# cvsp-lab/ICLR2025_3D-MOM

Hardware: AMD Instinct MI355X
Metric: 4DGS train-steps/sec @200k Gaussians, 960×540, 60 frames; render FPS (higher is better)
Workload: dtype f32

## Files before the change

### iclr2025_3d-mom_amd/csrc/hexplane.hip

```cpp
#include "hexplane_dev.h"

namespace {

template <int C> constexpr int kGroups = 64 / C;
template <int C> constexpr unsigned kRowB = 4u * C;
template <int C> constexpr int kPad = C == 16 ? 1 : 0;
constexpr int kChunk = 32;
template <int C> constexpr int kPerGroup = kChunk / kGroups<C>;
template <int C> constexpr int kRecs = kChunk * 6 + kPad<C> * kGroups<C>;
template <int C> __device__ __forceinline__ constexpr int rec_idx(int pt, int p) { return pt * 6 + p + kPad<C> * (pt / kPerGroup<C>); }

template <int C> __device__ __forceinline__ float group_sum(float v)
{
#pragma unroll
    for (int d = C / 2; d >= 1; d >>= 1) v += __shfl_xor(v, d);
    return v;
}

template <int C> __device__ __forceinline__ void norm_coords_fwd(const HexArgs& a, const float* __restrict__ xyz, int g, float c[4])
{
    if constexpr (C == 32) norm_coords_fwd32(a, xyz, g, c);
    else norm_coords(a, xyz, g, c);
}

template <int C>
__global__ void __launch_bounds__(256) hexplane_fwd_kernel(HexArgs a, const float* __restrict__ xyz, float* __restrict__ feat)
{
    const int ch = threadIdx.x & (C - 1);
    const long long unit = (long long)blockIdx.x * (256 / C) + threadIdx.x / C;
    const int gi = (int)(unit / a.levels), lvl = (int)(unit % a.levels);
    if (gi >= a.P) return;
    const int g = a.order ? (int)a.order[gi] : gi;
    float c[4];
    norm_coords_fwd<C>(a, xyz, g, c);
    float prod = 1.f;
#pragma unroll
    for (int p = 0; p < 6; p++) {
        const int ca = kCombA[p], cb = kCombB[p];
        const int Wd = a.res[lvl][ca], Hd = a.res[lvl][cb];
        const PlaneSample s = make_sample(c[ca], c[cb], Wd, Hd);
        const float* __restrict__ pl = a.planes[lvl][p];
        float v = 0.f;
        if (s.i00 >= 0) v += pl[(size_t)s.i00 * C + ch] * s.w00;
        if (s.i01 >= 0) v += pl[(size_t)s.i01 * C + ch] * s.w01;
        if (s.i10 >= 0) v += pl[(size_t)s.i10 * C + ch] * s.w10;
        if (s.i11 >= 0) v += pl[(size_t)s.i11 * C + ch] * s.w11;
        prod = prod * v;
    }
    feat[(size_t)g * (a.levels * C) + lvl * C + ch] = prod;
}

template <int C>
__global__ void __launch_bounds__(256)
hexplane_bwd_kernel(HexArgs a, const float* __restrict__ xyz, const float* __restrict__ dfeat, float* __restrict__ dxyz)
{
    const int ch = threadIdx.x & (C - 1);
    const long long unit = (long long)blockIdx.x * (256 / C) + threadIdx.x / C;
    const int g = (int)(unit / a.levels), lvl = (int)(unit % a.levels);
    if (g >= a.P) return;
    float c[4];
    norm_coords(a, xyz, g, c);
    PlaneSample s[6];
    float v[6], t00[6], t01[6], t10[6], t11[6];
#pragma unroll
    for (int p = 0; p < 6; p++) {
        const int ca = kCombA[p], cb = kCombB[p];
        s[p] = make_sample(c[ca], c[cb], a.res[lvl][ca], a.res[lvl][cb]);
        const float* __restrict__ pl = a.planes[lvl][p];
        t00[p] = s[p].i00 >= 0 ? pl[(size_t)s[p].i00 * C + ch] : 0.f;
        t01[p] = s[p].i01 >= 0 ? pl[(size_t)s[p].i01 * C + ch] : 0.f;
        t10[p] = s[p].i10 >= 0 ? pl[(size_t)s[p].i10 * C + ch] : 0.f;
        t11[p] = s[p].i11 >= 0 ? pl[(size_t)s[p].i11 * C + ch] : 0.f;
        float acc = 0.f;
        acc += t00[p] * s[p].w00;
        acc += t01[p] * s[p].w01;
        acc += t10[p] * s[p].w10;
        acc += t11[p] * s[p].w11;
        v[p] = acc;
    }
    const float go = dfeat[(size_t)g * (a.levels * C) + lvl * C + ch];
    float pre[7], suf[7];
    pre[0] = 1.f;
#pragma unroll
    for (int p = 0; p < 6; p++) pre[p + 1] = pre[p] * v[p];
    suf[6] = 1.f;
#pragma unroll
    for (int p = 5; p >= 0; p--) suf[p] = suf[p + 1] * v[p];
    float gc[3] = {0.f, 0.f, 0.f};
#pragma unroll
    for (int p = 0; p < 6; p++) {
        const float gv = go * pre[p] * suf[p + 1];
        float* __restrict__ gp = a.grads[lvl][p];
        if (s[p].i00 >= 0) atomicAdd(&gp[(size_t)s[p].i00 * C + ch], gv * s[p].w00);
        if (s[p].i01 >= 0) atomicAdd(&gp[(size_t)s[p].i01 * C + ch], gv * s[p].w01);
        if (s[p].i10 >= 0) atomicAdd(&gp[(size_t)s[p].i10 * C + ch], gv * s[p].w10);
        if (s[p].i11 >= 0) atomicAdd(&gp[(size_t)s[p].i11 * C + ch], gv * s[p].w11);
        const float x0 = (float)s[p].ixn, y0 = (float)s[p].iyn, x1 = x0 + 1.f, y1 = y0 + 1.f;
        float gix = 0.f, giy = 0.f;
        gix -= t00[p] * (y1 - s[p].iy) * gv;
        giy -= t00[p] * (x1 - s[p].ix) * gv;
        gix += t01[p] * (y1 - s[p].iy) * gv;
        giy -= t01[p] * (s[p].ix - x0) * gv;
        gix -= t10[p] * (s[p].iy - y0) * gv;
        giy += t10[p] * (x1 - s[p].ix) * gv;
        gix += t11[p] * (s[p].iy - y0) * gv;
        giy += t11[p] * (s[p].ix - x0) * gv;
        const int ca = kCombA[p], cb = kCombB[p];
        if (ca < 3) gc[ca] += gix * s[p].gx_mul;
        if (cb < 3) gc[cb] += giy * s[p].gy_mul;
    }
    if (dxyz) {
#pragma unroll
        for (int k = 0; k < 3; k++) {
            const float tot = group_sum<C>(gc[k]) * (2.0f / (a.a1[k] - a.a0[k]));
            if (ch == 0) atomicAdd(&dxyz[3 * g + k], tot);
        }
    }
}



template <int C>
__device__ __forceinline__ void make_rec_fwd(float cx, float cy, int Wd, int Hd, uint4& O, float4& Wt)
{
    float gxm, gym;
    const float ix = unnorm_clip(cx, Wd, gxm), iy = unnorm_clip(cy, Hd, gym);
    const int x0 = (int)floorf(ix), y0 = (int)floorf(iy);
    const unsigned o00 = (unsigned)(y0 * Wd + x0) * kRowB<C>, sx = (x0 + 1 < Wd) ? kRowB<C> : 0u, sy = (y0 + 1 < Hd) ? (unsigned)Wd * kRowB<C> : 0u;
    const float bx = ix - (float)x0, by = iy - (float)y0, ax = 1.f - bx, ay = 1.f - by;
    O = make_uint4(o00, o00 + sx, o00 + sy, o00 + sy + sx);
    Wt = make_float4(ax * ay, bx * ay, ax * by, bx * by);
}

template <int C>
__global__ void __launch_bounds__(256)
hexplane_fwd4_kernel(HexArgs a, int nchunks, const float* __restrict__ xyz, float* __restrict__ feat)
{
    __shared__ uint4 s_off[4][kRecs<C>];
    __shared__ float4 s_wt[4][kRecs<C>];
    const int lane = threadIdx.x & 63, ch = lane & (C - 1), q = lane / C, wv = threadIdx.x >> 6;
    const int lvl = blockIdx.y;
    const int wave = (blockIdx.x * 256 + threadIdx.x) >> 6, nwaves = (gridDim.x * 256) >> 6;
    for (int chunk = wave; chunk < nchunks; chunk += nwaves) {
        const int gi = chunk * kChunk + lane;
        const int g_mine = (lane < kChunk && gi < a.P) ? (a.order ? (int)a.order[gi] : gi) : -1;
        __builtin_amdgcn_wave_barrier();
        if (g_mine >= 0) {
            float c[4];
            norm_coords_fwd<C>(a, xyz, g_mine, c);
#pragma unroll
            for (int p = 0; p < 6; p++)
                make_rec_fwd<C>(c[kCombA[p]], c[kCombB[p]], a.res[lvl][kCombA[p]], a.res[lvl][kCombB[p]], s_off[wv][rec_idx<C>(lane, p)],
                                s_wt[wv][rec_idx<C>(lane, p)]);
        }
        __builtin_amdgcn_wave_barrier();
        const int npts = min(kChunk, a.P - chunk * kChunk);
        const int n_grp = max(0, min(kPerGroup<C>, npts - kPerGroup<C> * q));
        for (int i = 0; i < n_grp; i++) {
            const int pt = kPerGroup<C> * q + i;
            const int g = __shfl(g_mine, pt);
            float prod = 1.f;
#pragma unroll
            for (int p = 0; p < 6; p++) {
                const uint4 o = s_off[wv][rec_idx<C>(pt, p)];
                const float4 w = s_wt[wv][rec_idx<C>(pt, p)];
                const float* __restrict__ pl = a.planes[lvl][p] + ch;
                float v = 0.f;
                v += ld_f32(pl, o.x) * w.x;
                v += ld_f32(pl, o.y) * w.y;
                v += ld_f32(pl, o.z) * w.z;
                v += ld_f32(pl, o.w) * w.w;
                prod = prod * v;
            }
            feat[(size_t)g * (a.levels * C) + lvl * C + ch] = prod;
        }
    }
}


template <int C>
__device__ __forceinline__ void make_rec5(float cx, float cy, int Wd, int Hd, unsigned row_off, float gsx, float gsy, uint4& R1, float4& R2)
{
    float gxm, gym;
    const float ix = unnorm_clip(cx, Wd, gxm), iy = unnorm_clip(cy, Hd, gym);
    const int x0 = (int)floorf(ix), y0 = (int)floorf(iy);
    R1 = make_uint4((unsigned)(y0 * Wd + x0) * kRowB<C>, (x0 + 1 < Wd) ? kRowB<C> : 0u, (y0 + 1 < Hd) ? (unsigned)Wd * kRowB<C> : 0u, row_off);
    R2 = make_float4(ix - (float)x0, iy - (float)y0, gxm != 0.f ? gsx : 0.f, gym != 0.f ? gsy : 0.f);
}

template <int C>
__global__ void __launch_bounds__(256, 4)
hexplane_bwd5_gather_kernel(HexArgs a, int nchunks, const float* __restrict__ xyz, const float* __restrict__ dfeat,
                            float* __restrict__ dxyz, const uint32_t* __restrict__ inv ,
                            float* __restrict__ gvbuf )
{
    __shared__ uint4 s_r1[4][kRecs<C>];
    __shared__ float4 s_r2[4][kRecs<C>];
    const int lane = threadIdx.x & 63, ch = lane & (C - 1), q = lane / C, wv = threadIdx.x >> 6;
    const int pj = lane & 31, hh = lane >> 5;
    const int lvl = blockIdx.y;
    const int wave = (blockIdx.x * 256 + threadIdx.x) >> 6, nwaves = (gridDim.x * 256) >> 6;
    const unsigned chb = (unsigned)ch * 4u;
    const size_t plane_floats = (size_t)a.P * C;
    float gscale[4];
#pragma unroll
    for (int k = 0; k < 3; k++) gscale[k] = ((float)(a.res[lvl][k] - 1) / 2.f) * (2.0f / (a.a1[k] - a.a0[k]));
    gscale[3] = 0.f;

    for (int chunk = wave; chunk < nchunks; chunk += nwaves) {
        const int gi = chunk * kChunk + pj;
        const int g_mine = gi < a.P ? (a.order ? (int)a.order[gi] : gi) : -1;
        __builtin_amdgcn_wave_barrier();
        if (g_mine >= 0) {
            float c[4];
            norm_coords(a, xyz, g_mine, c);
            unsigned pos[3];
#pragma unroll
            for (int k = 0; k < 3; k++) pos[k] = inv[((size_t)k * a.levels + lvl) * a.P + g_mine] * (2u * kRowB<C>);
#pragma unroll
            for (int r = 0; r < 3; r++) {
                const int p0 = r, p1 = 3 + r;
                const int ca = hh ? kCombA[p1] : kCombA[p0], cb = hh ? kCombB[p1] : kCombB[p0];
                const int slot = hh ? order_slot_of_plane(p1) : order_slot_of_plane(p0);
                uint4 R1; float4 R2;
                make_rec5<C>(c[ca], c[cb], a.res[lvl][ca], a.res[lvl][cb], pos[slot], gscale[ca], gscale[cb], R1, R2);
                s_r1[wv][rec_idx<C>(pj, 3 * hh + r)] = R1;
                s_r2[wv][rec_idx<C>(pj, 3 * hh + r)] = R2;
            }
        }
        __builtin_amdgcn_wave_barrier();
        const int npts = min(kChunk, a.P - chunk * kChunk);
        const int n_grp = max(0, min(kPerGroup<C>, npts - kPerGroup<C> * q));
        const int pt0 = kPerGroup<C> * q;
        float t00[6], t01[6], t10[6], t11[6];
        float go = 0.f;
        float dx_mine[3] = {0.f, 0.f, 0.f};
        auto fetch = [&](int i) {
            const int ng = __shfl(g_mine, pt0 + i);
#pragma unroll
            for (int p = 0; p < 6; p++) {
                const uint4 R1 = s_r1[wv][rec_idx<C>(pt0 + i, p)];
                const float* __restrict__ pl = a.planes[lvl][p];
                const unsigned o = R1.x + chb;
                t00[p] = ld_f32(pl, o);
                t01[p] = ld_f32(pl, o + R1.y);
                t10[p] = ld_f32(pl, o + R1.z);
                t11[p] = ld_f32(pl, o + R1.y + R1.z);
            }
            go = dfeat[(size_t)ng * (a.levels * C) + lvl * C + ch];
        };
        if (n_grp > 0) fetch(0);
        for (int i = 0; i < n_grp; i++) {
            float v[6], dgx[6], dgy[6];
#pragma unroll
            for (int p = 0; p < 6; p++) {
                const float4 R2 = s_r2[wv][rec_idx<C>(pt0 + i, p)];
                const float d0 = t01[p] - t00[p], d1 = t11[p] - t10[p];
                const float tx0 = __builtin_fmaf(R2.x, d0, t00[p]), tx1 = __builtin_fmaf(R2.x, d1, t10[p]);
                const float dy = tx1 - tx0;
                v[p] = __builtin_fmaf(R2.y, dy, tx0);
                dgx[p] = __builtin_fmaf(R2.y, d1 - d0, d0) * R2.z;
                dgy[p] = dy * R2.w;
            }
            const float gcur = go;
            const int icur = i;
            if (i + 1 < n_grp) fetch(i + 1);
            float pre[7], suf[7];
            pre[0] = 1.f;
#pragma unroll
            for (int p = 0; p < 6; p++) pre[p + 1] = pre[p] * v[p];
            suf[6] = 1.f;
#pragma unroll
            for (int p = 5; p >= 0; p--) suf[p] = suf[p + 1] * v[p];
            float gc[3] = {0.f, 0.f, 0.f};
#pragma unroll
            for (int p = 0; p < 6; p++) {
                const float gv = gcur * (pre[p] * suf[p + 1]);
                const int ca = kCombA[p], cb = kCombB[p];
                float* __restrict__ dst = gvbuf + ((size_t)order_slot_of_plane(p) * a.levels + lvl) * 2 * plane_floats + ((p == 2 || p == 4 || p == 5) ? C : 0);
                *reinterpret_cast<float*>(reinterpret_cast<char*>(dst) + (s_r1[wv][rec_idx<C>(pt0 + icur, p)].w + chb)) = gv;
                gc[ca] = __builtin_fmaf(gv, dgx[p], gc[ca]);
                if (cb < 3) gc[cb] = __builtin_fmaf(gv, dgy[p], gc[cb]);
            }
            if (dxyz) {
#pragma unroll
                for (int k = 0; k < 3; k++) {
                    const float tot = group_sum<C>(gc[k]);
                    if (ch == icur) dx_mine[k] = tot;
                }
            }
        }
        if (dxyz) {
            const int gp = __shfl(g_mine, pt0 + (ch & (kPerGroup<C> - 1)));
            if (ch < n_grp && gp >= 0) {
#pragma unroll
                for (int k = 0; k < 3; k++) atomicAdd(&dxyz[3 * gp + k], dx_mine[k]);
            }
        }
    }
}

constexpr int kBatch5s = 16;
constexpr int kRec5s = 4 + 4 + 4 + 2;
template <int C> constexpr int kSlots5s = 64 + kPad<C> * kGroups<C>;

template <int C, bool CROWS>
__global__ void __launch_bounds__(256)
hexplane_bwd5_scatter_kernel(HexArgs a, int per_group, const float* __restrict__ xyz,
                             const uint32_t* __restrict__ order , const float* __restrict__ gvbuf,
                             const float* __restrict__ lines, LineTab lt)
{
    static_assert(!CROWS || C == 32, "the line table and the common-factor gather are 32 channels");
    extern __shared__ float s_dyn5[];
    constexpr int kS = kSlots5s<C>, kPer = kS * kRec5s;
    float* s_line = s_dyn5 + 4 * kPer;
    const int lane = threadIdx.x & 63, ch = lane & (C - 1), q = lane / C, wv = threadIdx.x >> 6;
    const int si = blockIdx.y, lvl = blockIdx.z;
    const int p = si == 0 ? 0 : (si == 1 ? 1 : 3), ca = si == 2 ? 1 : 0, cb = si == 0 ? 1 : 2;
    const int pt = si == 0 ? 2 : (si == 1 ? 5 : 4);
    const bool ride_on_b = si == 1;
    const int cs = ride_on_b ? cb : ca;
    const int Wd = a.res[lvl][ca], Hd = a.res[lvl][cb], Ws = a.res[lvl][cs];
    float* __restrict__ gp = a.grads[lvl][p] + ch;
    const size_t plane_floats = (size_t)a.P * C;
    const float* __restrict__ src_s = gvbuf + ((size_t)si * a.levels + lvl) * (CROWS ? 1 : 2) * plane_floats + ch;
    const float* __restrict__ src_t = src_s + C;
    constexpr int kRowF = CROWS ? C : 2 * C;
    const float* __restrict__ plane_v = a.planes[lvl][p] + ch;
    const uint32_t* __restrict__ ord = order + ((size_t)si * a.levels + lvl) * a.P;
    const float lo_a = a.a0[ca], sc_a = 2.0f / (a.a1[ca] - a.a0[ca]), lo_b = a.a0[cb], sc_b = 2.0f / (a.a1[cb] - a.a0[cb]);
    float* __restrict__ my_line = s_line + ch;
    const float* __restrict__ my_lval = CROWS ? lines + lt.off[lvl][cs] + ch : nullptr;
    for (int i = threadIdx.x; i < Ws * C; i += 256) s_line[i] = 0.f;
    __syncthreads();
    float tv[4] = {0.f, 0.f, 0.f, 0.f}, lv[2] = {0.f, 0.f};

    int pid[4] = {-1, -1, -1, -1};
    float pacc[4] = {0.f, 0.f, 0.f, 0.f};
    int lpid[2] = {-1, -1};
    float lacc[2] = {0.f, 0.f};
    int prev_cell = -1, prev_row = -1;
    const long long grp = ((long long)blockIdx.x * 4 + wv) * kGroups<C> + q;
    const long long r_begin = grp * per_group;
    const int r_end = (int)(r_begin + per_group < (long long)a.P ? r_begin + per_group : (long long)a.P);
    float* rec = s_dyn5 + wv * kPer;
    int4* w_ids = reinterpret_cast<int4*>(rec);
    float4* w_ws = reinterpret_cast<float4*>(rec + 4 * kS);
    float4* w_rd = reinterpret_cast<float4*>(rec + 8 * kS);
    int2* w_rid = reinterpret_cast<int2*>(rec + 12 * kS);
    const int sl0 = (C + kPad<C>) * q;
    for (long long base_ll = r_begin; base_ll < r_end; base_ll += C) {
        const int base = (int)base_ll;
        const int npts = min(C, r_end - base);
        __builtin_amdgcn_wave_barrier();
        {
            const bool on = ch < npts;
            const int g = (int)ord[base + (on ? ch : 0)];
            const float cx = norm_coord(xyz[3 * g + ca], lo_a, sc_a), cy = norm_coord(xyz[3 * g + cb], lo_b, sc_b);
            float gxm, gym;
            const float ix = unnorm_clip(cx, Wd, gxm), iy = unnorm_clip(cy, Hd, gym);
            const int x0 = (int)floorf(ix), y0 = (int)floorf(iy);
            const bool hx = x0 + 1 < Wd, hy = y0 + 1 < Hd;
            const int o00 = (y0 * Wd + x0) * C;
            const float bx = ix - (float)x0, by = iy - (float)y0, ax = 1.f - bx, ay = 1.f - by;
            const int ids[4] = {o00, hx ? o00 + C : -2, hy ? o00 + Wd * C : -2, (hx && hy) ? o00 + Wd * C + C : -2};
            const float ws[4] = {ax * ay, bx * ay, ax * by, bx * by};
            const bool sx1 = x0 & 1, sy1 = y0 & 1;
            const int i0 = sx1 ? ids[1] : ids[0], i1 = sx1 ? ids[0] : ids[1], i2 = sx1 ? ids[3] : ids[2], i3 = sx1 ? ids[2] : ids[3];
            const float f0 = sx1 ? ws[1] : ws[0], f1 = sx1 ? ws[0] : ws[1], f2 = sx1 ? ws[3] : ws[2], f3 = sx1 ? ws[2] : ws[3];
            const int r0 = ride_on_b ? y0 : x0;
            const bool hr = ride_on_b ? hy : hx;
            const float bw = ride_on_b ? by : bx, aw = 1.f - bw;
            const bool odd = r0 & 1;
            const int ra = r0 * C, rb = hr ? (r0 + 1) * C : -2;
            const int cell = (hx && hy) ? o00 : -2 - ch, row = hr ? r0 : -2 - ch;
            int pc = __shfl_up(cell, 1), pr = __shfl_up(row, 1);
            if (ch == 0) { pc = prev_cell; pr = prev_row; }
            const int flag = (cell != pc ? 1 : 0) | (row != pr ? 2 : 0);
            prev_cell = __shfl(cell, C * q + max(npts, 1) - 1);
            prev_row = __shfl(row, C * q + max(npts, 1) - 1);
            if (on) {
                w_ids[sl0 + ch] = make_int4(sy1 ? i2 : i0, sy1 ? i3 : i1, sy1 ? i0 : i2, sy1 ? i1 : i3);
                w_ws[sl0 + ch] = make_float4(sy1 ? f2 : f0, sy1 ? f3 : f1, sy1 ? f0 : f2, sy1 ? f1 : f3);
                w_rd[sl0 + ch] = make_float4(odd ? bw : aw, odd ? aw : bw, __int_as_float(flag), 0.f);
                w_rid[sl0 + ch] = make_int2(odd ? rb : ra, odd ? ra : rb);
            }
        }
        __builtin_amdgcn_wave_barrier();
        const int nbatched = C > kBatch5s ? npts : 1;
        for (int b0 = 0; b0 < nbatched; b0 += kBatch5s) {
            float val[kBatch5s], vat[kBatch5s];
#pragma unroll
            for (int j = 0; j < kBatch5s; j++) {
                const int r = min(b0 + j, npts - 1);
                val[j] = src_s[(size_t)(base + r) * kRowF];
                vat[j] = CROWS ? 0.f : src_t[(size_t)(base + r) * kRowF];
            }
#pragma unroll
            for (int j = 0; j < kBatch5s; j++) {
                if (b0 + j >= npts) continue;
                const int sl = sl0 + b0 + j;
                const float4 w4 = w_ws[sl];
                const float4 rd = w_rd[sl];
                const int flag = __float_as_int(rd.z);
                const float ws[4] = {w4.x, w4.y, w4.z, w4.w};
                const float lw[2] = {rd.x, rd.y};
                float g_space = val[j], g_time = vat[j];
                if (CROWS) {
                    if (flag & 2) {
                        const int2 r2 = w_rid[sl];
                        const int lid[2] = {r2.x, r2.y};
#pragma unroll
                        for (int k = 0; k < 2; k++) {
                            if (lid[k] != lpid[k] && lid[k] >= 0) {
                                if (lpid[k] >= 0) atomicAdd(&my_line[lpid[k]], lacc[k]);
                                lpid[k] = lid[k];
                                lacc[k] = 0.f;
                                lv[k] = my_lval[lid[k]];
                            }
                        }
                    }
                    g_space = val[j] * (lw[0] * lv[0] + lw[1] * lv[1]);
                }
                if (flag & 1) {
                    const int4 id4 = w_ids[sl];
                    const int ids[4] = {id4.x, id4.y, id4.z, id4.w};
#pragma unroll
                    for (int k = 0; k < 4; k++) {
                        if (ids[k] == pid[k]) {
                            pacc[k] = __builtin_fmaf(g_space, ws[k], pacc[k]);
                        } else if (ids[k] >= 0) {
                            if (pid[k] >= 0) atomicAdd(&gp[pid[k]], pacc[k]);
                            pid[k] = ids[k];
                            pacc[k] = g_space * ws[k];
                            if (CROWS) tv[k] = plane_v[ids[k]];
                        }
                    }
                } else {
#pragma unroll
                    for (int k = 0; k < 4; k++) pacc[k] = __builtin_fmaf(g_space, ws[k], pacc[k]);
                }
                if (CROWS) {
                    g_time = val[j] * (ws[0] * tv[0] + ws[1] * tv[1] + ws[2] * tv[2] + ws[3] * tv[3]);
#pragma unroll
                    for (int k = 0; k < 2; k++) lacc[k] = __builtin_fmaf(g_time, lw[k], lacc[k]);
                } else if (flag & 2) {
                    const int2 r2 = w_rid[sl];
                    const int lid[2] = {r2.x, r2.y};
#pragma unroll
                    for (int k = 0; k < 2; k++) {
                        if (lid[k] == lpid[k]) {
                            lacc[k] = __builtin_fmaf(g_time, lw[k], lacc[k]);
                        } else if (lid[k] >= 0) {
                            if (lpid[k] >= 0) atomicAdd(&my_line[lpid[k]], lacc[k]);
                            lpid[k] = lid[k];
                            lacc[k] = g_time * lw[k];
                        }
                    }
                } else {
#pragma unroll
                    for (int k = 0; k < 2; k++) lacc[k] = __builtin_fmaf(g_time, lw[k], lacc[k]);
                }
            }
        }
    }
#pragma unroll
    for (int k = 0; k < 4; k++)
        if (pid[k] >= 0) atomicAdd(&gp[pid[k]], pacc[k]);
#pragma unroll
    for (int k = 0; k < 2; k++)
        if (lpid[k] >= 0) atomicAdd(&my_line[lpid[k]], lacc[k]);
    __syncthreads();
    int t0, t1;
    float wt0, wt1;
    time_sample(a.time, a.res[lvl][3], t0, t1, wt0, wt1);
    float* __restrict__ gt = a.grads[lvl][pt];
    for (int i = threadIdx.x; i < Ws * C; i += 256) {
        const float sv = s_line[i];
        if (sv != 0.f) {
            if (t0 >= 0) atomicAdd(&gt[(size_t)t0 * Ws * C + i], sv * wt0);
            if (t1 >= 0) atomicAdd(&gt[(size_t)t1 * Ws * C + i], sv * wt1);
        }
    }
}

__device__ __forceinline__ unsigned spread16(unsigned x)
{
    x &= 0xFFFFu;
    x = (x | (x << 8)) & 0x00FF00FFu;
    x = (x | (x << 4)) & 0x0F0F0F0Fu;
    x = (x | (x << 2)) & 0x33333333u;
    x = (x | (x << 1)) & 0x55555555u;
    return x;
}
__global__ void __launch_bounds__(256)
plane_key_kernel(HexArgs a, int ca, int cb, int Wd, int Hd, const float* __restrict__ xyz, unsigned* __restrict__ keys,
                 unsigned* __restrict__ idx)
{
    const int i = blockIdx.x * 256 + threadIdx.x;
    if (i >= a.P) return;
    const float cx = norm_coord(xyz[3 * i + ca], a.a0[ca], 2.0f / (a.a1[ca] - a.a0[ca]));
    const float cy = norm_coord(xyz[3 * i + cb], a.a0[cb], 2.0f / (a.a1[cb] - a.a0[cb]));
    float gm;
    const int x0 = (int)floorf(unnorm_clip(cx, Wd, gm)), y0 = (int)floorf(unnorm_clip(cy, Hd, gm));
    keys[i] = spread16((unsigned)x0) | (spread16((unsigned)y0) << 1);
    idx[i] = (unsigned)i;
}
__global__ void __launch_bounds__(256)
invert_perm_kernel(int n, const unsigned* __restrict__ order, unsigned* __restrict__ order_out, unsigned* __restrict__ inv)
{
    const int i = blockIdx.x * 256 + threadIdx.x;
    if (i >= n) return;
    const unsigned g = order[i];
    order_out[i] = g;
    inv[g] = (unsigned)i;
}

}

int mom_sort_pairs_u32(int n, int bits, unsigned* keys[2], unsigned* vals[2], unsigned* counts, hipStream_t s);
size_t mom_sort_pairs_counts_bytes(int n);

static bool channels_ok(const MomHexPlane* hp) { return hp->channels == 32 || hp->channels == 16; }

static bool planes_fit32(const MomHexPlane* hp, unsigned rowbytes)
{
    static const int ca[6] = {0, 0, 0, 1, 1, 2}, cb[6] = {1, 2, 3, 2, 3, 3};
    for (int l = 0; l < hp->levels; l++)
        for (int p = 0; p < 6; p++)
            if ((unsigned long long)hp->res[l][ca[p]] * (unsigned long long)hp->res[l][cb[p]] * rowbytes >= (1ull << 31)) return false;
    return true;
}

template <int C>
static int hexplane_forward(const MomHexPlane* hp, int P, const float* xyz, const float* times, float time, const uint32_t* order,
                            float* feat, hipStream_t s)
{
    HexArgs a;
    fill_args(hp, P, times, time, order, false, &a);
    if (!times && planes_fit32(hp, kRowB<C>)) {
        const int nchunks = (P + kChunk - 1) / kChunk;
        int blocks = (nchunks + 3) / 4;
        if (blocks > 8192) blocks = 8192;
        hipLaunchKernelGGL(hexplane_fwd4_kernel<C>, dim3(blocks, hp->levels), dim3(256), 0, s, a, nchunks, xyz, feat);
        return hipGetLastError() == hipSuccess ? MOM_OK : MOM_ELAUNCH;
    }
    constexpr int kUnits = 256 / C;
    const long long units = (long long)P * hp->levels;
    hipLaunchKernelGGL(hexplane_fwd_kernel<C>, dim3((unsigned)((units + kUnits - 1) / kUnits)), dim3(256), 0, s, a, xyz, feat);
    return hipGetLastError() == hipSuccess ? MOM_OK : MOM_ELAUNCH;
}

extern "C" int mom_hexplane_forward(const MomHexPlane* hp, int P, const float* xyz, const float* times, float time,
                                    const uint32_t* order, float* feat, mom_stream_t stream)
{
    if (!hp || !channels_ok(hp) || hp->levels < 1 || hp->levels > 4 || P < 0) return MOM_EINVAL;
    if (P == 0) return MOM_OK;
    if (!xyz || !feat) return MOM_EINVAL;
    MomProfScope ps(MOM_P_HEX_FWD, (hipStream_t)stream);
    return hp->channels == 32 ? hexplane_forward<32>(hp, P, xyz, times, time, order, feat, (hipStream_t)stream)
                              : hexplane_forward<16>(hp, P, xyz, times, time, order, feat, (hipStream_t)stream);
}

extern "C" size_t mom_hexplane_orders_scratch_bytes(int P)
{
    const size_t n = (size_t)(P > 0 ? P : 1);
    return 4 * mom_align_up(n * 4) + mom_align_up(mom_sort_pairs_counts_bytes(P)) + MOM_ALIGN;
}

extern "C" int mom_hexplane_orders(const MomHexPlane* hp, int P, const float* xyz, uint32_t* order, uint32_t* inverse, void* scratch,
                                   mom_stream_t stream)
{
    if (!hp || hp->levels < 1 || hp->levels > 4 || P < 0) return MOM_EINVAL;
    if (P == 0) return MOM_OK;
    if (!xyz || !order || !inverse || !scratch) return MOM_EINVAL;
    hipStream_t s = (hipStream_t)stream;
    HexArgs a;
    fill_args(hp, P, nullptr, 0.f, nullptr, false, &a);
    const size_t n = (size_t)P;
    char* base = mom_align_ptr(scratch);
    unsigned* keys[2]; unsigned* vals[2];
    keys[0] = (unsigned*)base; base += mom_align_up(n * 4);
    keys[1] = (unsigned*)base; base += mom_align_up(n * 4);
    vals[0] = (unsigned*)base; base += mom_align_up(n * 4);
    vals[1] = (unsigned*)base; base += mom_align_up(n * 4);
    unsigned* counts = (unsigned*)base;
    const int axes[3][2] = {{0, 1}, {0, 2}, {1, 2}};
    for (int si = 0; si < 3; si++)
        for (int l = 0; l < hp->levels; l++) {
            const int ca = axes[si][0], cb = axes[si][1], Wd = hp->res[l][ca], Hd = hp->res[l][cb];
            if (Wd < 1 || Hd < 1 || Wd > 65536 || Hd > 65536) return MOM_EINVAL;
            int bits = 0;
            while ((1 << bits) < (Wd > Hd ? Wd : Hd)) bits++;
            hipLaunchKernelGGL(plane_key_kernel, dim3((P + 255) / 256), dim3(256), 0, s, a, ca, cb, Wd, Hd, xyz, keys[0], vals[0]);
            const int cur = mom_sort_pairs_u32(P, 2 * bits, keys, vals, counts, s);
            if (cur < 0) return cur;
            const size_t off = ((size_t)si * hp->levels + l) * n;
            hipLaunchKernelGGL(invert_perm_kernel, dim3((P + 255) / 256), dim3(256), 0, s, P, vals[cur], order + off, inverse + off);
        }
    return hipGetLastError() == hipSuccess ? MOM_OK : MOM_ELAUNCH;
}

size_t mom_hexplane_lines_bytes(const MomHexPlane* hp);
int mom_launch_hexplane_gather6(const MomHexPlane* hp, int P, const float* xyz, float time, const uint32_t* order, const float* dfeat,
                                float* dxyz, const uint32_t* plane_inverse, float* gvbuf, float* lines, bool lines_ready, hipStream_t s);
extern "C" int mom_deform_field_supported(const MomHexPlane* hp);

static size_t gv_bytes(const MomHexPlane* hp, int P) { return mom_align_up((size_t)6 * (size_t)P * (size_t)hp->levels * (size_t)hp->channels * sizeof(float)); }

extern "C" size_t mom_hexplane_backward_scratch_bytes(const MomHexPlane* hp, int P)
{
    if (!hp || !channels_ok(hp) || P <= 0) return MOM_ALIGN;
    return gv_bytes(hp, P) + mom_hexplane_lines_bytes(hp) + MOM_ALIGN;
}

static int hexplane_backward(const MomHexPlane* hp, int P, const float* xyz, const float* times, float time,
                             const uint32_t* order, const float* dfeat, float* dxyz, const uint32_t* plane_order,
                             const uint32_t* plane_inverse, void* scratch, const void* field_scratch, mom_stream_t stream);

extern "C" int mom_hexplane_backward(const MomHexPlane* hp, int P, const float* xyz, const float* times, float time,
                                     const uint32_t* order, const float* dfeat, float* dxyz, const uint32_t* plane_order,
                                     const uint32_t* plane_inverse, void* scratch, mom_stream_t stream)
{
    return hexplane_backward(hp, P, xyz, times, time, order, dfeat, dxyz, plane_order, plane_inverse, scratch, nullptr, stream);
}

extern "C" int mom_hexplane_backward_lines(const MomHexPlane* hp, int P, const float* xyz, float time, const uint32_t* order,
                                           const float* dfeat, float* dxyz, const uint32_t* plane_order,
                                           const uint32_t* plane_inverse, void* scratch, const void* field_scratch,
                                           mom_stream_t stream)
{
    if (!field_scratch || !plane_order || !plane_inverse || !scratch) return MOM_EINVAL;
    if (!hp || hp->channels != 32) return MOM_EINVAL;
    return hexplane_backward(hp, P, xyz, nullptr, time, order, dfeat, dxyz, plane_order, plane_inverse, scratch, field_scratch, stream);
}

template <int C>
static int hexplane_backward_launch(const MomHexPlane* hp, const HexArgs& a, const float* xyz, const float* dfeat, float* dxyz,
                                    const uint32_t* plane_order, const uint32_t* plane_inverse, void* scratch, const void* field_scratch,
                                    hipStream_t s)
{
    const int P = a.P;
    constexpr int kUnits = 256 / C;
    constexpr int kSGroups = 4 * kGroups<C>;
    int wmax = 0;
    for (int l = 0; l < hp->levels; l++)
        for (int k = 0; k < 3; k++)
            if (hp->res[l][k] > wmax) wmax = hp->res[l][k];
    const size_t lds_s = sizeof(float) * ((size_t)4 * kSlots5s<C> * kRec5s + (size_t)wmax * C);
    const bool fits32 = (unsigned long long)P * (2ull * kRowB<C>) < (1ull << 32);
    if (!a.times && plane_order && plane_inverse && scratch && lds_s <= 160 * 1024 && fits32 && planes_fit32(hp, kRowB<C>)) {
        if (!mom_lds_limit<hexplane_bwd5_scatter_kernel<C, false>>(160 * 1024)) return MOM_ELAUNCH;
        float* gvbuf = (float*)mom_align_ptr(scratch);
        constexpr int kGather5MaxBlocks = 1536;
        static const int blocks_s = mom_env_int("MOM_HEX_SBLOCKS", 512, 1, 1 << 16);
        const int groups = blocks_s * kSGroups;
        int per_group = (P + groups - 1) / groups;
        per_group = ((per_group + C - 1) / C) * C;
        const int sblocks = (int)(((long long)P + (long long)per_group * kSGroups - 1) / ((long long)per_group * kSGroups));
        LineTab lt;
        line_table(hp, &lt);
        if constexpr (C == 32) {
            if (mom_env_int("MOM_HEX_GATHER", 6, 5, 6) == 6 && mom_deform_field_supported(hp)) {
                if (!mom_lds_limit<hexplane_bwd5_scatter_kernel<32, true>>(160 * 1024)) return MOM_ELAUNCH;
                float* lines = field_scratch ? (float*)mom_align_ptr(const_cast<void*>(field_scratch))
                                             : (float*)mom_align_ptr((char*)gvbuf + gv_bytes(hp, P));
                int rc = mom_launch_hexplane_gather6(hp, P, xyz, a.time, a.order, dfeat, dxyz, plane_inverse, gvbuf, lines, field_scratch != nullptr, s);
                if (rc) return rc;
                hipLaunchKernelGGL((hexplane_bwd5_scatter_kernel<32, true>), dim3(sblocks, 3, hp->levels), dim3(256), lds_s, s, a, per_group, xyz,
                                   plane_order, gvbuf, lines, lt);
                return hipGetLastError() == hipSuccess ? MOM_OK : MOM_ELAUNCH;
            }
        }
        const int nchunks = (P + kChunk - 1) / kChunk;
        int blocks = (nchunks + 3) / 4;
        if (blocks > kGather5MaxBlocks) blocks = kGather5MaxBlocks;
        hipLaunchKernelGGL(hexplane_bwd5_gather_kernel<C>, dim3(blocks, hp->levels), dim3(256), 0, s, a, nchunks, xyz, dfeat, dxyz, plane_inverse,
                           gvbuf);
        if (hipGetLastError() != hipSuccess) return MOM_ELAUNCH;
        hipLaunchKernelGGL((hexplane_bwd5_scatter_kernel<C, false>), dim3(sblocks, 3, hp->levels), dim3(256), lds_s, s, a, per_group, xyz,
                           plane_order, gvbuf, (const float*)nullptr, lt);
        return hipGetLastError() == hipSuccess ? MOM_OK : MOM_ELAUNCH;
    }
    const long long units = (long long)P * hp->levels;
    hipLaunchKernelGGL(hexplane_bwd_kernel<C>, dim3((unsigned)((units + kUnits - 1) / kUnits)), dim3(256), 0, s, a, xyz, dfeat, dxyz);
    return hipGetLastError() == hipSuccess ? MOM_OK : MOM_ELAUNCH;
}

static int hexplane_backward(const MomHexPlane* hp, int P, const float* xyz, const float* times, float time,
                             const uint32_t* order, const float* dfeat, float* dxyz, const uint32_t* plane_order,
                             const uint32_t* plane_inverse, void* scratch, const void* field_scratch, mom_stream_t stream)
{
    if (!hp || !channels_ok(hp) || hp->levels < 1 || hp->levels > 4 || P < 0) return MOM_EINVAL;
    if (P == 0) return MOM_OK;
    if (!xyz || !dfeat) return MOM_EINVAL;
    HexArgs a;
    fill_args(hp, P, times, time, order, true, &a);
    for (int l = 0; l < hp->levels; l++)
        for (int p = 0; p < 6; p++)
            if (!a.planes[l][p] || !a.grads[l][p]) return MOM_EINVAL;
    MomProfScope ps(MOM_P_HEX_BWD, (hipStream_t)stream);
    return hp->channels == 32
               ? hexplane_backward_launch<32>(hp, a, xyz, dfeat, dxyz, plane_order, plane_inverse, scratch, field_scratch, (hipStream_t)stream)
               : hexplane_backward_launch<16>(hp, a, xyz, dfeat, dxyz, plane_order, plane_inverse, scratch, field_scratch, (hipStream_t)stream);
}
```

Baseline: 1166.

## Add optional software pipelining and timing stamps to hexplane scatter backward kernel

Restructures the bwd5 scatter kernel so that, behind a compile-time HEX_SCATTER_PIPE level, gradient rows for the next batch and the order and xyz gathers for the next chunk are loaded into a second register set while the current batch is consumed. This is meant to hide global load latency. The default level is 0, which keeps the old batch-of-16 load-then-consume flow, but two other changes always apply: the launch bounds now add an occupancy hint (5 or 4 blocks per CU), and loads and atomics go through unsigned byte offsets via ld_f32 and lane_off. It also adds optional SCATTER_STAMPS instrumentation that records per-wave s_memtime segment timings and copies them to the host.

```diff
diff --git a/iclr2025_3d-mom_amd/csrc/hexplane.hip b/iclr2025_3d-mom_amd/csrc/hexplane.hip
--- a/iclr2025_3d-mom_amd/csrc/hexplane.hip
+++ b/iclr2025_3d-mom_amd/csrc/hexplane.hip
@@ -300,12 +300,33 @@
     }
 }
 
-constexpr int kBatch5s = 16;
+#ifndef HEX_SCATTER_PIPE
+#define HEX_SCATTER_PIPE 0
+#endif
+constexpr int kPipe5s = HEX_SCATTER_PIPE;
+static_assert(kPipe5s >= 0 && kPipe5s <= 3, "HEX_SCATTER_PIPE is 0 .. 3");
+constexpr int kBatch5s = kPipe5s >= 1 ? 8 : 16;
+template <int C, bool CROWS> constexpr int kPipeOf5s = (C == 32 && !CROWS && kPipe5s > 1) ? 1 : kPipe5s;
 constexpr int kRec5s = 4 + 4 + 4 + 2;
+
+#ifdef SCATTER_STAMPS
+#if HEX_SCATTER_PIPE != 0
+#error "-DSCATTER_STAMPS goes with -DHEX_SCATTER_PIPE=0: the stamps' registers on top of a second register set spill to scratch"
+#endif
+enum { kStClear, kStOrder, kStPos, kStRows0, kStRows1, kStConsume, kStFlush, kStAck, kStSegs };
+constexpr int kStampWaves = 4 * 3 * 512 * 4;
+__device__ unsigned g_scatter_stamps[kStampWaves][kStSegs];
+#define ST_CLOSE(seg) do { __builtin_amdgcn_sched_barrier(0); const unsigned t_ = (unsigned)__builtin_amdgcn_s_memtime(); \
+                           st_acc[seg] += t_ - st_last; st_last = t_; __builtin_amdgcn_sched_barrier(0); } while (0)
+#define ST_WAIT(before, seg) do { ST_CLOSE(before); __builtin_amdgcn_s_waitcnt(0x0F70);  ST_CLOSE(seg); } while (0)
+#else
+#define ST_CLOSE(seg) do { } while (0)
+#define ST_WAIT(before, seg) do { } while (0)
+#endif
 template <int C> constexpr int kSlots5s = 64 + kPad<C> * kGroups<C>;
 
 template <int C, bool CROWS>
-__global__ void __launch_bounds__(256)
+__global__ void __launch_bounds__(256, C == 32 ? 5 : 4)
 hexplane_bwd5_scatter_kernel(HexArgs a, int per_group, const float* __restrict__ xyz,
                              const uint32_t* __restrict__ order , const float* __restrict__ gvbuf,
                              const float* __restrict__ lines, LineTab lt)
@@ -321,18 +342,57 @@
     const bool ride_on_b = si == 1;
     const int cs = ride_on_b ? cb : ca;
     const int Wd = a.res[lvl][ca], Hd = a.res[lvl][cb], Ws = a.res[lvl][cs];
-    float* __restrict__ gp = a.grads[lvl][p] + ch;
+    float* __restrict__ gp = a.grads[lvl][p];
+    auto lane_off = [&](int idx) { return (unsigned)(idx + ch) * 4u; };
+    auto add_f32 = [&](float* base, int idx, float v) { atomicAdd(reinterpret_cast<float*>(reinterpret_cast<char*>(base) + lane_off(idx)), v); };
     const size_t plane_floats = (size_t)a.P * C;
-    const float* __restrict__ src_s = gvbuf + ((size_t)si * a.levels + lvl) * (CROWS ? 1 : 2) * plane_floats + ch;
-    const float* __restrict__ src_t = src_s + C;
-    constexpr int kRowF = CROWS ? C : 2 * C;
-    const float* __restrict__ plane_v = a.planes[lvl][p] + ch;
+    const float* __restrict__ src = gvbuf + ((size_t)si * a.levels + lvl) * (CROWS ? 1 : 2) * plane_floats;
+    constexpr unsigned kRowBy = (CROWS ? C : 2 * C) * 4;
+    const float* __restrict__ plane_v = a.planes[lvl][p];
     const uint32_t* __restrict__ ord = order + ((size_t)si * a.levels + lvl) * a.P;
     const float lo_a = a.a0[ca], sc_a = 2.0f / (a.a1[ca] - a.a0[ca]), lo_b = a.a0[cb], sc_b = 2.0f / (a.a1[cb] - a.a0[cb]);
     float* __restrict__ my_line = s_line + ch;
-    const float* __restrict__ my_lval = CROWS ? lines + lt.off[lvl][cs] + ch : nullptr;
+    const float* __restrict__ my_lval = CROWS ? lines + lt.off[lvl][cs] : nullptr;
+#ifdef SCATTER_STAMPS
+    unsigned st_acc[kStSegs] = {}, st_last = (unsigned)__builtin_amdgcn_s_memtime();
+#endif
+    constexpr int kB = kBatch5s, kNb = C / kB;
+    constexpr int kPipe = kPipeOf5s<C, CROWS>;
+    constexpr bool kRowsAhead = kPipe >= 1, kChunkAhead = kPipe >= 2, kEarly = kPipe >= 3;
+    static_assert(kNb >= 1 && (!kRowsAhead || kNb % 2 == 0), "the two register sets alternate inside a chunk");
+    const long long grp = ((long long)blockIdx.x * 4 + wv) * kGroups<C> + q;
+    const long long r_begin = grp * per_group;
+    const int r_end = (int)(r_begin + per_group < (long long)a.P ? r_begin + per_group : (long long)a.P);
+    const bool some = r_begin < (long long)a.P;
+    float val[kRowsAhead ? 2 : 1][kB], vat[kRowsAhead ? 2 : 1][kB];
+    const unsigned off_last = (unsigned)(r_end - 1) * kRowBy + (unsigned)ch * 4u;
+    auto request_rows = [&](int set, int row0) {
+        const unsigned off0 = (unsigned)row0 * kRowBy + (unsigned)ch * 4u;
+#pragma unroll
+        for (int j = 0; j < kB; j++) {
+            const unsigned o = min(off0 + j * kRowBy, off_last);
+            val[set][j] = ld_f32(src, o);
+            vat[set][j] = CROWS ? 0.f : ld_f32(src, o + C * 4);
+        }
+    };
+    int g_ahead = 0;
+    float xa_ahead = 0.f, xb_ahead = 0.f;
+    auto request_first = [&]() {
+        if (some) {
+            if (kChunkAhead) g_ahead = (int)ord[min((int)r_begin + ch, r_end - 1)];
+            if (kRowsAhead) request_rows(0, (int)r_begin);
+        }
+    };
+    if (kEarly) request_first();
     for (int i = threadIdx.x; i < Ws * C; i += 256) s_line[i] = 0.f;
     __syncthreads();
+    ST_CLOSE(kStClear);
+    if (!kEarly) request_first();
+    if (kChunkAhead) {
+        ST_WAIT(kStConsume, kStOrder);
+        xa_ahead = xyz[3 * g_ahead + ca];
+        xb_ahead = xyz[3 * g_ahead + cb];
+    }
     float tv[4] = {0.f, 0.f, 0.f, 0.f}, lv[2] = {0.f, 0.f};
 
     int pid[4] = {-1, -1, -1, -1};
@@ -340,9 +400,6 @@
     int lpid[2] = {-1, -1};
     float lacc[2] = {0.f, 0.f};
     int prev_cell = -1, prev_row = -1;
-    const long long grp = ((long long)blockIdx.x * 4 + wv) * kGroups<C> + q;
-    const long long r_begin = grp * per_group;
-    const int r_end = (int)(r_begin + per_group < (long long)a.P ? r_begin + per_group : (long long)a.P);
     float* rec = s_dyn5 + wv * kPer;
     int4* w_ids = reinterpret_cast<int4*>(rec);
     float4* w_ws = reinterpret_cast<float4*>(rec + 4 * kS);
@@ -355,8 +412,19 @@
         __builtin_amdgcn_wave_barrier();
         {
             const bool on = ch < npts;
-            const int g = (int)ord[base + (on ? ch : 0)];
-            const float cx = norm_coord(xyz[3 * g + ca], lo_a, sc_a), cy = norm_coord(xyz[3 * g + cb], lo_b, sc_b);
+            float xa, xb;
+            if (kChunkAhead) {
+                ST_WAIT(kStConsume, kStPos);
+                xa = xa_ahead;
+                xb = xb_ahead;
+            } else {
+                const int g = (int)ord[base + (on ? ch : 0)];
+                ST_WAIT(kStConsume, kStOrder);
+                xa = xyz[3 * g + ca];
+                xb = xyz[3 * g + cb];
+                ST_WAIT(kStConsume, kStPos);
+            }
+            const float cx = norm_coord(xa, lo_a, sc_a), cy = norm_coord(xb, lo_b, sc_b);
             float gxm, gym;
             const float ix = unnorm_clip(cx, Wd, gxm), iy = unnorm_clip(cy, Hd, gym);
             const int x0 = (int)floorf(ix), y0 = (int)floorf(iy);
@@ -387,17 +455,24 @@
             }
         }
         __builtin_amdgcn_wave_barrier();
-        const int nbatched = C > kBatch5s ? npts : 1;
-        for (int b0 = 0; b0 < nbatched; b0 += kBatch5s) {
-            float val[kBatch5s], vat[kBatch5s];
-#pragma unroll
-            for (int j = 0; j < kBatch5s; j++) {
-                const int r = min(b0 + j, npts - 1);
-                val[j] = src_s[(size_t)(base + r) * kRowF];
-                vat[j] = CROWS ? 0.f : src_t[(size_t)(base + r) * kRowF];
-            }
-#pragma unroll
-            for (int j = 0; j < kBatch5s; j++) {
+        const bool more = base + C < r_end;
+#pragma unroll
+        for (int bi = 0; bi < kNb; bi++) {
+            const int b0 = bi * kB, set = kRowsAhead ? (bi & 1) : 0;
+            if (b0 >= npts) break;
+            if (!kRowsAhead) request_rows(0, base + b0);
+            else if (base + b0 + kB < r_end) request_rows(set ^ 1, base + b0 + kB);
+            if (kChunkAhead && more) {
+                if (bi == 0) g_ahead = (int)ord[min(base + C + ch, r_end - 1)];
+                if (bi == 1) {
+                    ST_WAIT(kStConsume, kStOrder);
+                    xa_ahead = xyz[3 * g_ahead + ca];
+                    xb_ahead = xyz[3 * g_ahead + cb];
+                }
+            }
+            ST_WAIT(kStConsume, bi == 0 ? kStRows0 : kStRows1);
+#pragma unroll
+            for (int j = 0; j < kB; j++) {
                 if (b0 + j >= npts) continue;
                 const int sl = sl0 + b0 + j;
                 const float4 w4 = w_ws[sl];
@@ -405,7 +480,7 @@
                 const int flag = __float_as_int(rd.z);
                 const float ws[4] = {w4.x, w4.y, w4.z, w4.w};
                 const float lw[2] = {rd.x, rd.y};
-                float g_space = val[j], g_time = vat[j];
+                float g_space = val[set][j], g_time = vat[set][j];
                 if (CROWS) {
                     if (flag & 2) {
                         const int2 r2 = w_rid[sl];
@@ -416,11 +491,11 @@
                                 if (lpid[k] >= 0) atomicAdd(&my_line[lpid[k]], lacc[k]);
                                 lpid[k] = lid[k];
                                 lacc[k] = 0.f;
-                                lv[k] = my_lval[lid[k]];
+                                lv[k] = ld_f32(my_lval, lane_off(lid[k]));
                             }
                         }
                     }
-                    g_space = val[j] * (lw[0] * lv[0] + lw[1] * lv[1]);
+                    g_space = val[set][j] * (lw[0] * lv[0] + lw[1] * lv[1]);
                 }
                 if (flag & 1) {
                     const int4 id4 = w_ids[sl];
@@ -430,10 +505,10 @@
                         if (ids[k] == pid[k]) {
                             pacc[k] = __builtin_fmaf(g_space, ws[k], pacc[k]);
                         } else if (ids[k] >= 0) {
-                            if (pid[k] >= 0) atomicAdd(&gp[pid[k]], pacc[k]);
+                            if (pid[k] >= 0) add_f32(gp, pid[k], pacc[k]);
                             pid[k] = ids[k];
                             pacc[k] = g_space * ws[k];
-                            if (CROWS) tv[k] = plane_v[ids[k]];
+                            if (CROWS) tv[k] = ld_f32(plane_v, lane_off(ids[k]));
                         }
                     }
                 } else {
@@ -441,7 +516,7 @@
                     for (int k = 0; k < 4; k++) pacc[k] = __builtin_fmaf(g_space, ws[k], pacc[k]);
                 }
                 if (CROWS) {
-                    g_time = val[j] * (ws[0] * tv[0] + ws[1] * tv[1] + ws[2] * tv[2] + ws[3] * tv[3]);
+                    g_time = val[set][j] * (ws[0] * tv[0] + ws[1] * tv[1] + ws[2] * tv[2] + ws[3] * tv[3]);
 #pragma unroll
                     for (int k = 0; k < 2; k++) lacc[k] = __builtin_fmaf(g_time, lw[k], lacc[k]);
                 } else if (flag & 2) {
@@ -464,9 +539,10 @@
             }
         }
     }
+    ST_CLOSE(kStConsume);
 #pragma unroll
     for (int k = 0; k < 4; k++)
-        if (pid[k] >= 0) atomicAdd(&gp[pid[k]], pacc[k]);
+        if (pid[k] >= 0) add_f32(gp, pid[k], pacc[k]);
 #pragma unroll
     for (int k = 0; k < 2; k++)
         if (lpid[k] >= 0) atomicAdd(&my_line[lpid[k]], lacc[k]);
@@ -482,7 +558,29 @@
             if (t1 >= 0) atomicAdd(&gt[(size_t)t1 * Ws * C + i], sv * wt1);
         }
     }
-}
+#ifdef SCATTER_STAMPS
+    ST_WAIT(kStFlush, kStAck);
+    const unsigned st_wave = ((blockIdx.z * 3 + blockIdx.y) * gridDim.x + blockIdx.x) * 4 + wv;
+    if (lane == 0 && st_wave < (unsigned)kStampWaves) {
+#pragma unroll
+        for (int k = 0; k < kStSegs; k++) g_scatter_stamps[st_wave][k] = st_acc[k];
+    }
+#endif
+}
+
+#ifdef SCATTER_STAMPS
+}
+extern "C" int mom_hexplane_scatter_stamps(unsigned* out, int clear)
+{
+    if (hipMemcpyFromSymbol(out, HIP_SYMBOL(g_scatter_stamps), sizeof(g_scatter_stamps)) != hipSuccess) return MOM_ELAUNCH;
+    if (clear) {
+        void* p = nullptr;
+        if (hipGetSymbolAddress(&p, HIP_SYMBOL(g_scatter_stamps)) != hipSuccess || hipMemset(p, 0, sizeof(g_scatter_stamps)) != hipSuccess) return MOM_ELAUNCH;
+    }
+    return MOM_OK;
+}
+namespace {
+#endif
 
 __device__ __forceinline__ unsigned spread16(unsigned x)
 {
```

Result: no change. 1166 (-0.1%).
